# nizepart/Research-and-Development-of-Kubernetes-Operator-for-Machine-Learning-Pipelines

Measured on AMD Instinct MI355X. Metric: served_tokens_per_sec, higher is better.
Workload: dtype bf16

## Files before the change

### research-and-development-of-kubernetes-operator-for-machine-learning-pipelines_amd/ops/csrc/bindings.cpp

```cpp
#include <cstdlib>
#include <string>
#include <torch/library.h>
#include <ATen/ATen.h>
#include <c10/hip/HIPStream.h>
#include <c10/core/DeviceGuard.h>
#include <cmath>

#include "launch.h"
#include "gemm_plan.h"

namespace {

using at::Tensor;

hipStream_t cur_stream() { return c10::hip::getCurrentHIPStream().stream(); }

void check_bf16(const Tensor& t, const char* name) {
  TORCH_CHECK(t.is_cuda(), name, " must be a GPU tensor");
  TORCH_CHECK(t.scalar_type() == at::kBFloat16, name, " must be bf16");
  TORCH_CHECK(t.is_contiguous(), name, " must be contiguous");
}
void check_i32(const Tensor& t, const char* name) {
  TORCH_CHECK(t.is_cuda(), name, " must be a GPU tensor");
  TORCH_CHECK(t.scalar_type() == at::kInt, name, " must be int32");
// ... 281 lines not shown
Tensor vmm_arena(int64_t bytes, int64_t device) {
  void* base = nullptr;
  long reserved = 0;
  std::shared_ptr<void> owner = mlop::vmm_reserve((long)bytes, (int)device, &base, &reserved);
  TORCH_CHECK(owner != nullptr, "hipMemAddressReserve failed");
  const at::Device dev(at::kCUDA, (int)device);
  return at::for_blob(base, {(int64_t)reserved})
      .deleter([owner, base](void*) mutable {
        mlop::vmm_forget(base);
        owner.reset();
      })
      .options(at::TensorOptions().dtype(at::kByte).device(dev))
      .target_device(dev)
      .make_tensor();
}

bool vmm_map_chunks(Tensor flat, int64_t region_stride, int64_t n_regions, int64_t chunk_bytes, int64_t first,
                    int64_t count, bool async) {
  return mlop::vmm_map_chunks(flat.data_ptr(), (long)region_stride, (int)n_regions, (long)chunk_bytes,
                              (long)first, (long)count, async);
}
int64_t vmm_chunks_ready(Tensor flat) { return mlop::vmm_chunks_ready(flat.data_ptr()); }
int64_t vmm_error(Tensor flat) { return mlop::vmm_error(flat.data_ptr()); }

template <int (*F)(int)>
int64_t knob(int64_t set) { return F((int)set); }

void gemm_dense_plan(int64_t variant, int64_t bm, int64_t bn, int64_t splits, int64_t stages) {
  mlop::gemm_dense_plan((int)variant, (int)bm, (int)bn, (int)splits, (int)stages);
}
void gemm_grouped_plan(int64_t bm, int64_t bn, int64_t stages, int64_t splits) {
  mlop::gemm_grouped_plan((int)bm, (int)bn, (int)stages, (int)splits);
}
bool gemm_sk_reserve() { return mlop::gemm_sk_reserve(); }

int64_t gemm_sk_workgroups(int64_t M, int64_t N, int64_t K) {
  return mlop::gemm_sk_workgroups(mlop::gemm_live_env(), (int)M, (int)N, (int)K);
}
int64_t gemm_workspace(int64_t M, int64_t N, int64_t K, int64_t epi) {
  return mlop::gemm_workspace_floats(mlop::gemm_live_env(), (int)M, (int)N, (int)K, epi == 2 ? 0 : (int)epi);
}
bool gemm_rope_supported(int64_t M, int64_t N, int64_t K) {
  return mlop::gemm_rope_supported(mlop::gemm_live_env(), (int)M, (int)N, (int)K);
}
bool w4_chain_ok(int64_t M, int64_t N, int64_t K) { return mlop::w4_chain_ok(mlop::gemm_live_env(), (int)M, (int)N, (int)K); }
bool mid_chain_ok(int64_t M, int64_t N, int64_t K, int64_t epi) {
  return mlop::mid_chain_ok(mlop::gemm_live_env(), (int)M, (int)N, (int)K, (int)epi);
}
bool gemv_chain_supported(int64_t M, int64_t N, int64_t K, int64_t epi) {
  return mlop::decode_chain_takes(mlop::gemm_live_env(), (int)M, (int)N, (int)K, (int)epi);
}
bool chain_ok(int64_t M, int64_t N, int64_t K, int64_t epi) {
  return mlop::chain_ok(mlop::gemm_live_env(), (int)M, (int)N, (int)K, (int)epi);
}
int64_t decode_chain_max_m() { return mlop::decode_chain_max_m(mlop::gemm_live_env()); }

std::vector<int64_t> route_list(const mlop::PlanEnv& env, int64_t M, int64_t N, int64_t K, int64_t op,
                                int64_t n_groups, int64_t rows_per_group) {
  mlop::GemmCall c;
  c.op = (int)op, c.M = (int)M, c.N = (int)N, c.K = (int)K;
  c.n_groups = (int)n_groups, c.rows_per_group = (int)rows_per_group;
  long f[mlop::kRouteFields];
  mlop::gemm_route_fields(mlop::gemm_route(env, c), f);
  return std::vector<int64_t>(f, f + mlop::kRouteFields);
}
std::vector<int64_t> gemm_route(int64_t M, int64_t N, int64_t K, int64_t op, int64_t n_groups, int64_t rows_per_group) {
  return route_list(mlop::gemm_live_env(), M, N, K, op, n_groups, rows_per_group);
}
std::vector<int64_t> gemm_route_env(int64_t M, int64_t N, int64_t K, int64_t op, int64_t cus, bool sk,
                                    int64_t n_groups, int64_t rows_per_group) {
  mlop::PlanEnv env = mlop::gemm_knobs();
  env.cus = (int)cus, env.sk = sk;
  return route_list(env, M, N, K, op, n_groups, rows_per_group);
}
std::vector<int64_t> gemm_tile_configs() {
  std::vector<int64_t> v;
  for (const mlop::TileCfg& t : mlop::kGemmTiles) v.insert(v.end(), {t.BM, t.BN, t.WM, t.WN, t.stages, t.setprio, t.rope});
  return v;
}

void check_a(const Tensor& a) {
  TORCH_CHECK(a.is_cuda() && a.scalar_type() == at::kBFloat16 && a.dim() == 2 && a.stride(1) == 1 &&
                  a.stride(0) % 8 == 0, "a must be bf16 [M, K], 16-B aligned rows");
}

mlop::RopeEpi rope_args(const Tensor& q_out, const Tensor& k_cache, const Tensor& v_cache, const Tensor& a,
                        const Tensor& w, const Tensor& pos, const Tensor& cos_sin, const Tensor& slots) {
  check_a(a);
  check_bf16(w, "w"); check_bf16(q_out, "q_out"); check_bf16(k_cache, "k_cache");
  check_bf16(v_cache, "v_cache"); check_i32(pos, "pos"); check_i32(slots, "slots");
  TORCH_CHECK(cos_sin.is_cuda() && cos_sin.scalar_type() == at::kFloat && cos_sin.is_contiguous(),
              "cos_sin f32");
  const int64_t M = a.size(0), K = a.size(1), N = w.size(0);
  TORCH_CHECK(w.dim() == 2 && w.size(1) == K && K % 64 == 0, "w [N, K], K % 64");
  TORCH_CHECK(q_out.dim() == 3 && k_cache.dim() == 4 && v_cache.dim() == 4, "ranks");
  const int64_t Hq = q_out.size(1), D = q_out.size(2), Hkv = k_cache.size(1), BS = k_cache.size(2);
  TORCH_CHECK(D == 128 && k_cache.size(3) == D && v_cache.sizes() == k_cache.sizes(),
              "head_dim 128; k and v [NB,Hkv,BS,D]");
  TORCH_CHECK(N == (Hq + 2 * Hkv) * D && q_out.size(0) == M, "qkv width / q_out rows");
  TORCH_CHECK(pos.numel() == M && slots.numel() == M, "pos/slots length");
  TORCH_CHECK(cos_sin.dim() == 2 && cos_sin.size(1) == D, "cos_sin [max_pos, D]");
  return mlop::RopeEpi{(uint16_t*)q_out.data_ptr(), (uint16_t*)k_cache.data_ptr(),
                       (uint16_t*)v_cache.data_ptr(), pos.data_ptr<int>(), cos_sin.data_ptr<float>(),
                       slots.data_ptr<int>(), (int)Hq, (int)Hkv, (int)BS};
}

// ... 517 lines not shown

TORCH_LIBRARY(mlop, m) {
  m.def("src_hash() -> str", &src_hash);
  m.def("device_delay(int us) -> ()", &device_delay);
  m.def("car_create(int rank, int world, int max_bytes, int device, bool split=False) -> int", &car_create);
  m.def("car_ipc_handle(int h) -> Tensor", &car_ipc_handle);
  m.def("car_open(int h, Tensor handles) -> ()", &car_open);
  m.def("car_all_reduce(int h, Tensor(a!) out, Tensor inp, bool two_shot=False) -> ()");
  m.def("car_all_reduce_add(int h, Tensor(a!) residual, Tensor inp) -> ()");
  m.def("car_broadcast(int h, Tensor(a!) buf, int root) -> ()");
  m.def("car_all_gather(int h, Tensor(a!) out, Tensor piece) -> ()");
  m.def("car_error(int h) -> int", &car_error);
  m.def("attn_fused_max_pairs(int n) -> int", &attn_fused_max_pairs);
  m.def("car_mem_mode(int h) -> int", &car_mem_mode);
  m.def("car_destroy(int h) -> ()", &car_destroy);
  m.def("chan_create(str name, int slots, int consumers) -> int", &chan_create);
  m.def("chan_open(str name) -> int", &chan_open);
  m.def("chan_send(int h, Tensor vals, int timeout_us) -> bool", &chan_send);
  m.def("chan_recv(int h, int consumer, Tensor(a!) out, int timeout_us) -> bool", &chan_recv);
  m.def("chan_unlink(str name) -> ()", &chan_unlink);
  m.def("chan_close(int h, bool unlink) -> ()", &chan_close);
  m.def("xg_create(str name, int world, int slots, int max_words) -> int", &xg_create);
  m.def("xg_open(str name, int rank) -> int", &xg_open);
  m.def("xg_exchange(int h, Tensor vals, Tensor(a!) out, Tensor(b!) counts, int timeout_us) -> bool", &xg_exchange);
  m.def("xg_close(int h) -> ()", &xg_close);
  m.def("ep_create(int rank, int world, int E, int k, int H, int tcap, int device) -> int", &ep_create);
  m.def("ep_ipc_handle(int h) -> Tensor", &ep_ipc_handle);
  m.def("ep_open(int h, Tensor handles) -> ()", &ep_open);
  m.def("ep_dispatch(int h, Tensor(a!) xp, Tensor(b!) offsets, Tensor x, Tensor topi) -> ()");
  m.def("ep_combine(int h, Tensor(a!) out, Tensor y, Tensor topw, Tensor topi) -> ()");
  m.def("ep_error(int h) -> int", &ep_error);
  m.def("ep_mem_mode(int h) -> int", &ep_mem_mode);
  m.def("ep_destroy(int h) -> ()", &ep_destroy);
  m.def("gemm_workspace(int M, int N, int K, int epi) -> int", &gemm_workspace);
  m.def("gemm_big_variant(int set=-1) -> int", &knob<mlop::gemm_big_variant>);
  m.def("gemm_half_tile(int set=-1) -> int", &knob<mlop::gemm_half_tile>);
  m.def("gemm_small_nt(int set=-1) -> int", &knob<mlop::gemm_small_nt>);
  m.def("attn_kv_nt(int set=-1) -> int", &knob<mlop::attn_kv_nt>);
  m.def("gemm_slab_nt(int set=-1) -> int", &knob<mlop::gemm_slab_nt>);
  m.def("gemm_rope_split(int set=-1) -> int", &knob<mlop::gemm_rope_split>);
  m.def("gemm_split_target(int set=-1) -> int", &knob<mlop::gemm_split_target>);
  m.def("gemm_grouped_narrow(int set=-1) -> int", &knob<mlop::gemm_grouped_narrow>);
  m.def("gemm_ws_max_m(int set=-1) -> int", &knob<mlop::gemm_ws_max_m>);
  m.def("decode_chain_max_m() -> int", &decode_chain_max_m);
  m.def("gemm_ws_plan(int rb, int u, int nt) -> ()", &gemm_ws_plan);
  m.def("gemm_ws_small_m(int set=-1) -> int", &knob<mlop::gemm_ws_small_m>);
  m.def("gemm_ws_rope_m(int set=-1) -> int", &knob<mlop::gemm_ws_rope_m>);
  m.def("flash_persist(int set=-1) -> int", &knob<mlop::flash_persist>);
  m.def("flash_stream(int set=-1) -> int", &knob<mlop::flash_stream>);
  m.def("gemm_grouped_balance(int set=-1) -> int", &knob<mlop::gemm_grouped_balance>);
  m.def("gemm_grouped_order(int set=-1) -> int", &knob<mlop::gemm_grouped_order>);
  m.def("moe_mid_tok(int set=-1) -> int", &knob<mlop::moe_mid_tok>);
  m.def("gemm_mid_chain(int set=-1) -> int", &knob<mlop::gemm_mid_chain>);
  m.def("mid_chain_ok(int M, int N, int K, int epi) -> bool", &mid_chain_ok);
  m.def("moe_mid_max_tokens(int set=-1) -> int", &knob<mlop::moe_mid_max_tokens>);
  m.def("gemm_grouped_plan(int bm, int bn, int stages, int splits) -> ()", &gemm_grouped_plan);
  m.def("gemm_dense_plan(int variant, int bm, int bn, int splits, int stages=0) -> ()", &gemm_dense_plan);
  m.def("gemm_small_stages(int set=-1) -> int", &knob<mlop::gemm_small_stages>);
  m.def("gemm_small_tile(int set=-1) -> int", &knob<mlop::gemm_small_tile>);
  m.def("gemm_sk_mode(int set=-1) -> int", &knob<mlop::gemm_sk_mode>);
  m.def("gemm_sk_reserve() -> bool", &gemm_sk_reserve);
  m.def("gemm_sk_workgroups(int M, int N, int K) -> int", &gemm_sk_workgroups);
  m.def("vmm_supported(int device) -> bool", &vmm_supported);
  m.def("vmm_granularity(int device) -> int", &vmm_granularity);
  m.def("vmm_arena(int bytes, int device) -> Tensor", &vmm_arena);
  m.def("vmm_map_chunks(Tensor flat, int region_stride, int n_regions, int chunk_bytes, int first, "
        "int count, bool async_) -> bool", &vmm_map_chunks);
  m.def("vmm_chunks_ready(Tensor flat) -> int", &vmm_chunks_ready);
  m.def("vmm_error(Tensor flat) -> int", &vmm_error);
  m.def("gemm_rope_supported(int M, int N, int K) -> bool", &gemm_rope_supported);
  m.def("w4_chain_ok(int M, int N, int K) -> bool", &w4_chain_ok);
  m.def("chain_ok(int M, int N, int K, int epi) -> bool", &chain_ok);
  m.def("gemm_route(int M, int N, int K, int op, int n_groups=0, int rows_per_group=0) -> int[]", &gemm_route);
  m.def("gemm_route_env(int M, int N, int K, int op, int cus, bool sk, int n_groups=0, int rows_per_group=0) -> int[]", &gemm_route_env);
  m.def("gemm_tile_configs() -> int[]", &gemm_tile_configs);
  m.def("gemm_res_ss(Tensor(a!) residual, Tensor a, Tensor w, Tensor(b!) ss_out) -> bool");
  m.def("gemm_rs(Tensor(a!) out, Tensor a, Tensor w, Tensor ss_in, float eps, int epi) -> bool");
  m.def("gemm_rs_rope(Tensor(a!) q_out, Tensor(b!) k_cache, Tensor(c!) v_cache, Tensor a, Tensor w, "
        "Tensor pos, Tensor cos_sin, Tensor slots, Tensor ss_in, float eps) -> bool");
  m.def("gemm_rope_cache(Tensor(a!) q_out, Tensor(b!) k_cache, Tensor(c!) v_cache, Tensor a, Tensor w, "
        "Tensor pos, Tensor cos_sin, Tensor slots) -> bool");
  m.def("gemm(Tensor(a!) out, Tensor a, Tensor w, Tensor(b!) ws, int epi) -> ()");
  m.def("grouped_gemm(Tensor(a!) out, Tensor a, Tensor w, Tensor offsets, int max_rows, "
        "int epi, Tensor? a_rows=None) -> ()");
  m.def("gemm_add_rmsnorm(Tensor(a!) out, Tensor(b!) residual, Tensor a, Tensor w, Tensor norm_w, "
        "Tensor(c!) ws, float eps) -> bool");
  m.def("gemv_chain_supported(int M, int N, int K, int epi) -> bool", &gemv_chain_supported);
  m.def("moe_route(Tensor(a!) topw, Tensor(b!) topi, Tensor logits) -> ()");
  m.def("moe_permute(Tensor(a!) xp, Tensor(b!) offsets, Tensor(c!) src, Tensor(d!) inv, Tensor x, "
        "Tensor topi, int e0, int n_local) -> ()");
  m.def("moe_combine(Tensor(a!) out, Tensor y, Tensor inv, Tensor topw) -> ()");
  m.def("moe_dispatch_small(Tensor(a!) topw, Tensor(b!) topi, Tensor(c!) xp, Tensor(d!) offsets, Tensor(e!) src, "
        "Tensor(f!) inv, Tensor(g!) x, Tensor router_w, int e0, int n_local, Tensor? pro_y=None, "
        "Tensor(h!)? pro_res=None, Tensor? pro_w=None, float pro_eps=0.0) -> bool");
  m.def("moe_dispatch_mid(Tensor(a!) topw, Tensor(b!) topi, Tensor(c!) offsets, Tensor(d!) arow, Tensor(e!) inv, "
        "Tensor(f!) x, Tensor router_w, int e0, int n_local, Tensor? pro_y=None, Tensor(g!)? pro_res=None, "
        "Tensor? pro_w=None, float pro_eps=0.0) -> bool");
  m.def("moe_down_combine_add_rmsnorm(Tensor(a!) out, Tensor(b!) residual, Tensor(c!) y, Tensor a, Tensor w2, "
        "Tensor offsets, int max_rows, Tensor inv, Tensor topw, Tensor norm_w, float eps) -> bool");
  m.def("moe_combine_add_rmsnorm(Tensor(a!) out, Tensor(b!) residual, Tensor y, Tensor inv, Tensor topw, "
        "Tensor norm_w, float eps) -> bool");
  m.def("argmax(Tensor(a!) out, Tensor logits) -> ()");
  m.def("sample(Tensor(a!) out, Tensor logits, Tensor temps, Tensor top_ks, Tensor top_ps, "
        "Tensor uniform, bool full) -> ()");
  m.def("penalty_reset(Tensor(a!) table, int slot, int vocab, Tensor prompt_ids, Tensor output_ids) -> ()");
  m.def("penalty_update(Tensor(a!) table, int vocab, Tensor slots, Tensor tokens) -> ()");
// ... 69 lines not shown
```

### research-and-development-of-kubernetes-operator-for-machine-learning-pipelines_amd/ops/csrc/gemm.hip

```cpp
#include "common.h"
#include "launch.h"
#include "gemm_plan.h"
#include "rope_epi.h"

#include <stdexcept>

namespace mlop {

enum { EPI_NONE = 0, EPI_SILU_MUL = 1, EPI_ROPE = 3 };
constexpr int kStages = 3;

__device__ __forceinline__ int swz(int r) { return (r >> 1) & 7; }



template <int AUX>
__device__ __forceinline__ u32x4 ld_b128(__amdgpu_buffer_rsrc_t rs, uint32_t off) {
  return __builtin_bit_cast(u32x4, __builtin_amdgcn_raw_buffer_load_b128(rs, off, 0, AUX));
}
template <int AUX>
__device__ __forceinline__ float ld_f32(__amdgpu_buffer_rsrc_t rs, uint32_t off) {
  return __uint_as_float(__builtin_amdgcn_raw_buffer_load_b32(rs, off, 0, AUX));
}

// ... 957 lines not shown
}

template <int EPI, bool GROUPED>
static void launch_route(const Route& rt, const uint16_t* A, int lda, const uint16_t* B, int ldb, uint16_t* C,
                         int ldc, float* ws, int M, int N, int K, const int* offsets, int n_groups,
                         hipStream_t st, const RopeEpi& re = RopeEpi{}) {
  if (rt.family == FAM_PP) return run_pp<EPI, GROUPED>(rt, A, lda, B, ldb, C, ldc, M, N, K, st, re, offsets, n_groups);
  if ((rt.family == FAM_W4 || rt.family == FAM_W4H) && !GROUPED) {
    if (!run_w4(EPI, A, lda, B, ldb, C, ldc, M, N, K, st, re, rt.BM)) throw std::runtime_error("gemm: four-wave launch refused");
    return;
  }
#define MLOP_GEMM(bm_, bn_, wm_, wn_, st_, prio_, rope_)                                                  \
  if constexpr (EPI != EPI_ROPE || rope_) {                                                               \
    if (rt.family == FAM_TILE && rt.BM == bm_ && rt.BN == bn_ && rt.WM == wm_ && rt.WN == wn_ &&          \
        rt.stages == st_ && rt.setprio == (int)prio_)                                                     \
      return run_cfg<bm_, bn_, wm_, wn_, EPI, GROUPED, st_, prio_>(A, lda, B, ldb, C, ldc, ws, M, N, K,   \
                                                                   rt.splits, rt.k_chunk, offsets,        \
                                                                   n_groups, rt.m_tiles, st, re);         \
  }
  MLOP_GEMM_TILES(MLOP_GEMM)
#undef MLOP_GEMM
  throw std::runtime_error("gemm: the route names no kernel built for this epilogue");
}

static GemmCall gemm_call(int op, int M, int N, int K, int lda, int ldb, int ldc) {
  GemmCall c;
  c.op = op, c.M = M, c.N = N, c.K = K, c.lda = lda, c.ldb = ldb, c.ldc = ldc;
  return c;
}

static void launch_splitk_reduce(int epi, uint16_t* C, int ldc, const float* ws, int M, int N, int splits,
                                 hipStream_t st, const int* m_valid = nullptr) {
  const int outw = epi == EPI_NONE ? N : N / 2;
  const long total = (long)M * (outw / 8);
  const int g = (int)std::min<long>((total + 255) / 256, 4096);
  if (epi == EPI_NONE) splitk_reduce_kernel<EPI_NONE><<<g, 256, 0, st>>>(C, ldc, ws, M, N, splits, m_valid);
  else splitk_reduce_kernel<EPI_SILU_MUL><<<g, 256, 0, st>>>(C, ldc, ws, M, N, splits, m_valid);
}

static void run_rope_route(const Route& rt, const void* A, int lda, const void* B, int M, int N, int K,
                           const RopeEpi& re, hipStream_t st) {
  if (rt.family == FAM_GEMV) return launch_gemv_rope(A, lda, B, M, N, K, re, st);
  if (rt.family == FAM_WS) return launch_ws(A, lda, B, K, nullptr, 0, M, N, K, EPI_ROPE, false, re, 0.f, st);
  if (rt.finish == FIN_ROPE_SLABS) {
    float* ws = sk_buf()->ws;
    launch_route<EPI_NONE, false>(rt, (const uint16_t*)A, lda, (const uint16_t*)B, K, nullptr, N, ws, M, N, K,
                                  nullptr, 0, st);
    return launch_rope_cache_slabs(re, ws, rt.splits, M, N, st);
  }
  launch_route<EPI_ROPE, false>(rt, (const uint16_t*)A, lda, (const uint16_t*)B, K, nullptr, 0, nullptr, M, N, K,
                                nullptr, 0, st, re);
}

bool launch_gemm_rope(const void* A, int lda, const void* B, int M, int N, int K, const RopeEpi& re,
                      hipStream_t st) {
  if (M == 0) return true;
  const Route rt = gemm_route(gemm_live_env(), gemm_call(OP_ROPE, M, N, K, lda, K, 0));
  if (!rt.ok()) return false;
  run_rope_route(rt, A, lda, B, M, N, K, re, st);
  return true;
}

bool launch_gemm_chain(int op, const void* A, int lda, const void* B, void* C, int ldc, int M, int N, int K,
                       const RopeEpi& rope, float* ss, float eps, hipStream_t st) {
  const PlanEnv env = gemm_live_env();
  const Route rt = gemm_route(env, gemm_call(op, M, N, K, lda, K, ldc));
  if (!rt.ok()) return false;
  const bool res = op == OP_CHAIN_RES_SS;
  const int epi = res ? EPI_NONE : op & 3;
  RopeEpi re = epi == EPI_ROPE ? rope : RopeEpi{};
  if (M <= decode_chain_max_m(env)) {
    if (rt.family == FAM_GEMV && res) launch_gemv_res(A, lda, B, C, M, N, K, st);
    else if (rt.family == FAM_GEMV) launch_gemv_rs(A, lda, B, C, ldc, M, N, K, epi, re, eps, st);
    else if (res) launch_ws(A, lda, B, K, C, N, M, N, K, 5, false, re, 0.f, st);
    else launch_ws(A, lda, B, K, C, ldc, M, N, K, epi, true, re, eps, st);
    return true;
  }
  if (res) {
    re.ss_out = ss;
    re.ss_tot = ss + (size_t)M * (N / 128);
  } else {
    re.ss_in = ss + (size_t)M * (K / 128);
    re.ss_inv_k = 1.f / (float)K;
    re.ss_eps = eps;
  }
  if (rt.family == FAM_W4 || rt.family == FAM_W4H)
    return run_w4(res ? 4 : epi | 8, (const uint16_t*)A, lda, (const uint16_t*)B, K, (uint16_t*)C, ldc, M, N, K, st, re, rt.BM);
  if (epi == EPI_ROPE) {
    if (rt.family == FAM_WS) launch_ws(A, lda, B, K, nullptr, 0, M, N, K, 3, true, re, eps, st);
    else run_rope_route(rt, A, lda, B, M, N, K, re, st);
    return true;
  }
  if (res) {
    float* ws = nullptr;
    int cus = 0;
    RopeEpi fin{};
    if (!gemm_sk_scratch(&ws, &fin.ss_cnt, &cus)) return false;
    fin.ss_tot = re.ss_tot;
    fin.mid_acq = env.mid_chain == 2;
    launch_route<EPI_NONE, false>(rt, (const uint16_t*)A, lda, (const uint16_t*)B, K, (uint16_t*)C, ldc, ws, M, N, K,
                                  nullptr, 0, st, fin);
    return true;
  }
  RopeEpi rs{};
  rs.ss_in = re.ss_in;
  rs.ss_inv_k = re.ss_inv_k;
  rs.ss_eps = eps;
  launch_route<EPI_SILU_MUL, false>(rt, (const uint16_t*)A, lda, (const uint16_t*)B, K, (uint16_t*)C, ldc, nullptr, M,
                                    N, K, nullptr, 0, st, rs);
  return true;
}

void launch_gemm(const void* A, int lda, const void* B, int ldb, void* C, int ldc, float* ws,
                 long ws_floats, int M, int N, int K, int epi, hipStream_t st) {
  if (M == 0) return;
  GemmCall c = gemm_call(epi, M, N, K, lda, ldb, ldc);
  c.ws_avail = ws_floats;
  const Route rt = gemm_route(gemm_live_env(), c);
// ... 72 lines not shown
```

### research-and-development-of-kubernetes-operator-for-machine-learning-pipelines_amd/ops/csrc/gemm_plan.cc

```cpp
#include "gemm_plan.h"

#include <algorithm>
#include <stddef.h>
#include <stdexcept>

namespace mlop {

namespace {
enum { EPI_NONE = 0, EPI_SILU_MUL = 1, EPI_ROPE = 3 };
enum { WS_NONE = 0, WS_SILU_MUL = 1, WS_ROPE = 3, WS_RES = 5 };
constexpr int kHeadD = 128;
constexpr int kGroupedSmallStages = 3;
}

static PlanEnv g_knobs;
PlanEnv& gemm_knobs() { return g_knobs; }

int gemm_split_target(int set) {
  if (set >= 1) g_knobs.split_target = set;
  return g_knobs.split_target;
}

int gemm_small_stages(int set) {
  if (set >= 0) g_knobs.small_stages = set;
// ... 406 lines not shown
    if (env.sk_on() && s > 1 && (size_t)s * M * N * 4 <= (size_t)kSkScratchFloats * 4) {
      p.splits = s;
      p.k_chunk = K / s;
    }
  }
  const Route r = resolve(env, p, M, N, K, true, false, false);
  return r.family == FAM_TILE && r.splits > 1 ? with_slabs(r, FIN_REDUCE, WS_SRC_SCRATCH, M, N) : r;
}

Route route_chain(const PlanEnv& env, const GemmCall& c, int lda, int ldc) {
  const int M = c.M, N = c.N, K = c.K;
  const int epi = c.op == OP_CHAIN_RES_SS ? EPI_NONE : c.op & 3;
  if (M <= decode_chain_max_m(env)) {
    if ((c.op == OP_CHAIN_RES_SS && ldc != N) || !decode_chain_takes(env, M, N, K, epi)) return refused();
    return simple(M <= env.gemv_chain_max_m ? FAM_GEMV : FAM_WS);
  }
  const Plan base = plan(env, M, N, K, false, 0, 0);
  const Plan p = epi == EPI_ROPE ? rope_split(env, base, K) : base;
  if (mid_chain_plan_ok(env, p, M, N, K, epi)) {
    if (epi == EPI_ROPE) {
      return ws_prefer(env, M, N, K, EPI_ROPE) ? simple(FAM_WS) : route_rope(env, c, lda);
    }
    if (c.op == OP_CHAIN_RS) return refused();
    Route r = resolve(env, p, M, N, K, false, false, false);
    if (epi == EPI_NONE) { r.ws_src = WS_SRC_SCRATCH; r.ws_floats = (long)r.splits * M * N; }
    return r;
  }
  if (!w4_chain_plan_ok(env, base, M, N, K) || !gemm_w4_ok(M, N, K, lda, K, ldc)) return refused();
  return w4_route(base.BM);
}

}

Route gemm_route(const PlanEnv& env, const GemmCall& c) {
  if (c.M <= 0) return refused();
  const bool silu = c.op == OP_SILU_MUL || c.op == OP_GROUPED_SILU || c.op == OP_CHAIN_RS_SILU;
  const int lda = c.lda ? c.lda : c.K, ldb = c.ldb ? c.ldb : c.K;
  const int ldc = c.ldc ? c.ldc : c.op == OP_ROPE || c.op == OP_CHAIN_RS_ROPE ? 0 : silu ? c.N / 2 : c.N;
  switch (c.op) {
    case OP_PLAIN:
    case OP_SILU_MUL: return route_plain(env, c, lda, ldb, ldc);
    case OP_ADD_RMSNORM: return route_add_rmsnorm(env, c, lda);
    case OP_ROPE: return route_rope(env, c, lda);
    case OP_CHAIN_RES_SS:
    case OP_CHAIN_RS:
    case OP_CHAIN_RS_SILU:
    case OP_CHAIN_RS_ROPE: return route_chain(env, c, lda, ldc);
    case OP_GROUPED:
    case OP_GROUPED_SILU: return route_grouped(env, c);
    default: throw std::runtime_error("gemm_route: unknown op");
  }
}

void gemm_route_fields(const Route& r, long out[kRouteFields]) {
  const long f[kRouteFields] = {r.family, r.tile,   r.BM,      r.BN,    r.WM,   r.WN,     r.stages, r.setprio,
                                r.splits, r.k_chunk, r.m_tiles, r.sk_d, r.sk_wgs, r.finish, r.ws_src, r.ws_floats};
  std::copy(f, f + kRouteFields, out);
}


static GemmCall call(int op, int M, int N, int K) {
  GemmCall c;
  c.op = op, c.M = M, c.N = N, c.K = K;
  return c;
}

bool gemm_rope_supported(const PlanEnv& e, int M, int N, int K) { return gemm_route(e, call(OP_ROPE, M, N, K)).ok(); }

bool w4_chain_ok(const PlanEnv& e, int M, int N, int K) {
  return M > 0 && w4_chain_plan_ok(e, plan(e, M, N, K, false, 0, 0), M, N, K);
}

bool mid_chain_ok(const PlanEnv& e, int M, int N, int K, int epi) {
  if (!mid_chain_rows(e, M, N, K)) return false;
  return mid_chain_plan_ok(e, epi == EPI_ROPE ? rope_plan(e, M, N, K) : plan(e, M, N, K, false, 0, 0), M, N, K, epi);
}

bool chain_ok(const PlanEnv& e, int M, int N, int K, int epi) {
  if (M <= decode_chain_max_m(e)) return decode_chain_takes(e, M, N, K, epi < 0 ? EPI_NONE : epi);
  if (M <= 64 && epi >= 0) return mid_chain_ok(e, M, N, K, epi);
  return w4_chain_ok(e, M, N, K);
}

long gemm_workspace_floats(const PlanEnv& e, int M, int N, int K, int epi) {
  const Route r = gemm_route(e, call(epi == EPI_SILU_MUL ? OP_SILU_MUL : OP_PLAIN, M, N, K));
  return r.ws_src == WS_SRC_CALLER ? r.ws_floats : 0;
}

int gemm_sk_workgroups(const PlanEnv& e, int M, int N, int K) {
  const Route r = gemm_route(e, call(OP_PLAIN, M, N, K));
  return r.family == FAM_PP ? r.sk_wgs : 0;
}

}
```

### research-and-development-of-kubernetes-operator-for-machine-learning-pipelines_amd/ops/csrc/gemm_plan.h

```cpp
#pragma once

#if defined(__HIP__) || defined(__HIPCC__)
#define MLOP_HD __host__ __device__
#else
#define MLOP_HD
#endif

namespace mlop {

constexpr int kBK = 64;
constexpr int kMaxSplits = 8;
constexpr int kSkMaxWg = 256;
constexpr long kSkScratchFloats = 2l * kSkMaxWg * 256 * 256;
constexpr int kSkMinIters = 16;
constexpr int sk_min_half() { return kSkMinIters / 2 > 1 ? kSkMinIters / 2 : 1; }

MLOP_HD inline int sk_choose_d(int T, int nk, int cus, int min_half) {
  const int r = T % cus;
  if (r == 0) return 0;
  float best = 0.9f * nk;
  int best_d = 0;
  const int dmax = cus / r < 32 ? cus / r : 32;
  for (int d = 2; d <= dmax; ++d) {
    if (nk % d || nk / d < min_half) continue;
    const float w = 0.04f * r * d;
    const float cost = nk / d + (w > 2.f ? w : 2.f) + 2.f * (d >= 3 ? d : d - 1) + 1.f;
    if (cost < best) {
      best = cost;
      best_d = d;
    }
  }
  return best_d;
}

struct PlanEnv {
  int cus = 0;
  bool sk = false;
  int small_tile = 1;
  int small_stages = 3;
  int big_variant = 5;
  int half_tile = 1;
  int grouped_narrow = 1;
  int split_target = 512;
  int rope_split_k = 2;
  int sk_mode = 1;
  int mid_chain = 0;
  int gp[4] = {-1, -1, -1, -1};
  int dp[5] = {-1, -1, -1, -1, 0};
  int ws_small_m = 8, ws_rope_m = 8, ws_max_m = 0;
  int gemv_max_m = 4, gemv_chain_max_m = 4;
  bool sk_on() const { return sk_mode && sk && cus > 0; }
};
PlanEnv& gemm_knobs();
PlanEnv gemm_live_env();
int gemm_small_tile(int set);
int gemm_small_stages(int set);
int gemm_big_variant(int set);
int gemm_half_tile(int set);
int gemm_grouped_narrow(int set);
int gemm_split_target(int set);
int gemm_rope_split(int set);
int gemm_sk_mode(int set);
int gemm_mid_chain(int set);
int gemm_ws_small_m(int set);
int gemm_ws_rope_m(int set);
int gemm_ws_max_m(int set);

enum GemmOp {
  OP_PLAIN = 0,
  OP_SILU_MUL = 1,
  OP_ADD_RMSNORM = 2,
  OP_ROPE = 3,
  OP_CHAIN_RES_SS = 4,
  OP_CHAIN_RS = 8,
  OP_CHAIN_RS_SILU = 9,
  OP_CHAIN_RS_ROPE = 11,
  OP_GROUPED = 16,
  OP_GROUPED_SILU = 17,
};

struct GemmCall {
  int op = OP_PLAIN;
  int M = 0, N = 0, K = 0;
  int lda = 0, ldb = 0, ldc = 0;
  int n_groups = 0, rows_per_group = 0;
  long ws_avail = -1;
  bool indirect = false;
};

enum GemmFamily { FAM_REFUSED = 0, FAM_GEMV, FAM_WS, FAM_TILE, FAM_PP, FAM_W4, FAM_W4H };
enum GemmFinish { FIN_NONE = 0, FIN_REDUCE, FIN_ADD_RMSNORM, FIN_ROPE_SLABS, FIN_RMSNORM };
enum GemmWsSrc { WS_SRC_NONE = 0, WS_SRC_CALLER, WS_SRC_SCRATCH };

#define MLOP_GEMM_TILES(X)       \
  X(16, 32, 1, 2, 8, false, 0)   \
  X(16, 32, 1, 2, 6, false, 0)   \
  X(16, 32, 1, 2, 4, false, 0)   \
  X(16, 64, 1, 2, 8, false, 0)   \
  X(16, 64, 1, 2, 6, false, 0)   \
  X(16, 64, 1, 2, 4, false, 0)   \
  X(32, 32, 1, 2, 8, false, 0)   \
  X(32, 32, 1, 2, 4, false, 0)   \
  X(32, 64, 1, 4, 6, false, 0)   \
  X(32, 64, 1, 4, 4, false, 0)   \
  X(64, 32, 1, 2, 4, false, 0)   \
  X(64, 64, 1, 4, 6, false, 0)   \
  X(64, 64, 1, 4, 4, false, 0)   \
  X(64, 64, 1, 4, 3, false, 0)   \
  X(128, 64, 2, 2, 5, false, 0)  \
  X(128, 64, 2, 2, 3, false, 0)  \
  X(256, 64, 4, 2, 3, false, 0)  \
  X(256, 128, 4, 2, 3, false, 1) \
  X(256, 256, 2, 4, 2, true, 1)  \
  X(256, 256, 2, 4, 2, false, 1)

struct TileCfg {
  int BM, BN, WM, WN, stages;
  bool setprio, rope;
};
#define MLOP_TILE_ENTRY(bm, bn, wm, wn, st, prio, rope) {bm, bn, wm, wn, st, prio, rope != 0},
constexpr TileCfg kGemmTiles[] = {MLOP_GEMM_TILES(MLOP_TILE_ENTRY)};
#undef MLOP_TILE_ENTRY
constexpr int kNumGemmTiles = sizeof(kGemmTiles) / sizeof(kGemmTiles[0]);

struct Route {
  int family = FAM_REFUSED;
  int tile = -1;
  int BM = 0, BN = 0, WM = 0, WN = 0, stages = 0, setprio = 0;
  int splits = 1, k_chunk = 0;
  int m_tiles = 0;
  int sk_d = 0, sk_wgs = 0;
  int finish = FIN_NONE;
  int ws_src = WS_SRC_NONE;
  long ws_floats = 0;
  bool ok() const { return family != FAM_REFUSED; }
};
constexpr int kRouteFields = 16;
void gemm_route_fields(const Route& r, long out[kRouteFields]);

Route gemm_route(const PlanEnv& env, const GemmCall& c);

void gemm_grouped_plan(int bm, int bn, int stages, int splits);
void gemm_dense_plan(int variant, int bm, int bn, int splits, int stages);

bool gemv_takes(const PlanEnv& e, int M, int N, int K, int epi);
bool gemv_chain_takes(const PlanEnv& e, int M, int N, int K, int epi);
bool gemv_grouped_takes(int M, int N, int K, int epi);
bool ws_takes(const PlanEnv& e, int M, int N, int K, int epi);
bool ws_prefer(const PlanEnv& e, int M, int N, int K, int epi);
int decode_chain_max_m(const PlanEnv& e);
bool decode_chain_takes(const PlanEnv& e, int M, int N, int K, int epi);
bool gemm_w4_ok(int M, int N, int K, int lda, int ldb, int ldc);
bool gemm_w4_split_ok(const PlanEnv& e, int T, int nk);
bool sk_halves_ok(const PlanEnv& e, long T, int nk);
bool gemm_rope_supported(const PlanEnv& e, int M, int N, int K);
bool w4_chain_ok(const PlanEnv& e, int M, int N, int K);
bool mid_chain_ok(const PlanEnv& e, int M, int N, int K, int epi);
bool chain_ok(const PlanEnv& e, int M, int N, int K, int epi);
long gemm_workspace_floats(const PlanEnv& e, int M, int N, int K, int epi);
int gemm_sk_workgroups(const PlanEnv& e, int M, int N, int K);

}
```

### research-and-development-of-kubernetes-operator-for-machine-learning-pipelines_amd/ops/csrc/gemm_w4.hip

```cpp
#include "common.h"
#include "launch.h"
#include "gemm_plan.h"
#include "gemm_w4_asm.h"

#include <type_traits>
#include <utility>

namespace mlop {

namespace {
enum { W4_NONE = 0, W4_SILU_MUL = 1, W4_ROPE = 3, W4_ADD_SS = 4, W4_RS = 8 };
using i32x4 = __attribute__((ext_vector_type(4))) int;
typedef __attribute__((address_space(3))) uint16_t lds_u16;

__device__ __forceinline__ i32x4 make_srd(const void* p) {
  const uint64_t a = (uint64_t)p;
  i32x4 r;
  r.x = __builtin_amdgcn_readfirstlane((int)(uint32_t)a);
  r.y = __builtin_amdgcn_readfirstlane((int)(uint32_t)(a >> 32));
  r.z = 0x7fffffff;
  r.w = 0x00020000;
  return r;
}

// ... 199 lines not shown
        const int tk = __hip_atomic_fetch_add(cnt + tt, 1, __ATOMIC_RELAXED, __HIP_MEMORY_SCOPE_AGENT);
        if (tk == 1) __hip_atomic_store(cnt + tt, 0, __ATOMIC_RELAXED, __HIP_MEMORY_SCOPE_AGENT);
        flag[0] = tk == 1;
      }
      __syncthreads();
      const int last = flag[0];
      __syncthreads();
      if (!last) break;
    }
    auto fetch = [&](auto I_, float (&v)[32]) {
      constexpr int I = decltype(I_)::value;
      read_block<I>(v);
      if (part) {
#pragma unroll
        for (int b4 = 0; b4 < 8; b4 += 4) {
          u32x4 o[4];
#pragma unroll
          for (int q4 = 0; q4 < 4; ++q4)
            o[q4] = __builtin_bit_cast(u32x4, __builtin_amdgcn_raw_buffer_load_b128(
                                                  rs_other, (uint32_t)(((I * 8 + b4 + q4) * 256 + tid) * 16), 0, 16 ));
#pragma unroll
          for (int q4 = 0; q4 < 4; ++q4)
#pragma unroll
            for (int e = 0; e < 4; ++e) v[4 * (b4 + q4) + e] += __uint_as_float(o[q4][e]);
        }
      }
      if constexpr (RS) {
        const float f = rsqrtf(rinv_lds[wid * 128 + 16 * I + (lane & 15)] * re.ss_inv_k + re.ss_eps);
#pragma unroll
        for (int e = 0; e < 32; ++e) v[e] *= f;
      }
    };
    const int odd = qd & 1, half = qd >> 1;
    auto swap_f = [&](const float* x, const float* y, float (&lo)[4], float (&hi)[4]) {
#pragma unroll
      for (int r = 0; r < 4; ++r) {
        const auto sw2 = __builtin_amdgcn_permlane16_swap(__float_as_uint(x[r]), __float_as_uint(y[r]), false, false);
        lo[r] = __uint_as_float(sw2[0]);
        hi[r] = __uint_as_float(sw2[1]);
      }
    };
    auto swap_pair = [&](const float* x, const float* y, u32x4& out) {
      float lo[4], hi[4];
      swap_f(x, y, lo, hi);
      out = u32x4{pack2(lo[0], lo[1]), pack2(lo[2], lo[3]), pack2(hi[0], hi[1]), pack2(hi[2], hi[3])};
    };
    if constexpr (BASE == W4_ROPE) {
      constexpr int D = 128, HALF = 64;
      const bool r_nt = (re.ws_nt & 8) != 0;
      auto put16 = [&](uint16_t* p, const u32x4& v) {
        if (r_nt) __builtin_nontemporal_store(v, reinterpret_cast<u32x4*>(p));
        else *reinterpret_cast<u32x4*>(p) = v;
      };
      const int head = (n0 + wn * 128) / D;
      const int n_rope = re.Hq + re.Hkv, n_all = re.Hq + 2 * re.Hkv;
      if (head >= n_all) {
      } else if (head >= n_rope) {
        const int kh = head - n_rope;
        int sl[NI];
#pragma unroll
        for (int I = 0; I < NI; ++I) {
          const int m = m0 + lr + I * 16;
          sl[I] = m < M ? re.slots[m] : -1;
        }
        auto vstore = [&](auto I_) {
          constexpr int I = decltype(I_)::value;
          float v[32];
          fetch(I_, v);
          u32x4 d[4];
#pragma unroll
          for (int pr = 0; pr < 4; ++pr) swap_pair(v + 8 * pr, v + 8 * pr + 4, d[pr]);
          const int slot = sl[I];
          if (slot < 0) return;
          uint16_t* dst = re.v_cache + (((size_t)(slot / re.BS) * re.Hkv + kh) * re.BS + slot % re.BS) * D;
#pragma unroll
          for (int pr = 0; pr < 4; ++pr)
            put16(dst + (2 * pr + odd) * 16 + 8 * half, d[pr]);
        };
        unroll<NI>(vstore);
      } else {
        const bool is_k = head >= re.Hq;
        int pp[NI], sl[NI];
#pragma unroll
        for (int I = 0; I < NI; ++I) {
          const int m = m0 + lr + I * 16;
          const bool ok = m < M;
          pp[I] = ok ? re.pos[m] : 0;
          sl[I] = ok && is_k ? re.slots[m] : -1;
        }
        const int c0 = 4 * qd;
        auto load_cs = [&](int I, float4 (&cs)[8]) {
          const float4* cr = reinterpret_cast<const float4*>(re.cos_sin + (size_t)pp[I] * D);
#pragma unroll
          for (int j = 0; j < 4; ++j) {
            cs[j] = cr[(j * 16 + c0) / 4];
            cs[4 + j] = cr[(HALF + j * 16 + c0) / 4];
          }
        };
        auto rstore = [&](auto I_, const float4 (&cs)[8], float4 (&nxt)[8]) {
          constexpr int I = decltype(I_)::value;
          if constexpr (I < NI - 1) load_cs(I + 1, nxt);
          float v[32];
          fetch(I_, v);
          float xo[4][4], yo[4][4];
#pragma unroll
          for (int j = 0; j < 4; ++j) {
            const float cv[4] = {cs[j].x, cs[j].y, cs[j].z, cs[j].w};
// ... 225 lines not shown
```

### research-and-development-of-kubernetes-operator-for-machine-learning-pipelines_amd/ops/csrc/launch.h

```cpp
#pragma once

#include <string>
#include <hip/hip_runtime.h>
#include <stdint.h>
#include <algorithm>
#include <memory>

namespace mlop {

void launch_rmsnorm(void* out, const void* x, const void* w, float eps, int M, int H,
                    hipStream_t st);
void launch_add_rmsnorm(void* out, void* residual, const void* x, const void* w, float eps, int M,
                        int H, hipStream_t st);
void launch_rope_cache(void* q_out, void* k_cache, void* v_cache, const void* qkv, const int* pos,
                       const float* cos_sin, const int* slots, int T, int Hq, int Hkv, int D,
                       int qkv_stride, int BS, hipStream_t st);
void launch_silu_mul(void* out, const void* x, int M, int I, int interleaved, hipStream_t st);
void launch_device_delay(long long ticks, hipStream_t st);
void launch_lora_shrink(const void* x, int ldx, const void* A, float* tmp, const int* tok_slot,
                        const int* slot_rank, int T, int K, int GR, int R, int S, hipStream_t st);
void launch_lora_expand_add(void* y, int ldy, const float* tmp, const void* B, const uint8_t* tile_group,
                            const int* tok_slot, const int* slot_rank, int T, int N, int GR, int R, int S,
                            hipStream_t st);
void launch_embedding(void* out, const void* table, const long* ids, int T, int H, long vocab_start,
                      long vocab_end, hipStream_t st);
void launch_paged_attention(void* out, float* part_o, float* part_ml, const void* q,
                            const void* kc, const void* vc, const int* bt, int bt_stride,
                            const int* tile_seq, const int* tile_q0, const int* q_start,
                            const int* q_len, const int* ctx_len, int num_tiles, int Hq, int Hkv,
                            float scale_log2, int part_tokens, int nparts, int num_blocks,
                            int* sem, int window, hipStream_t st);
void launch_rope_cache_fp8(void* q_out, void* k_cache, void* v_cache, void* k_scale, void* v_scale,
                           const void* qkv, const int* pos, const float* cos_sin, const int* slots, int T,
                           int Hq, int Hkv, int qkv_stride, int BS, hipStream_t st);
void launch_paged_attention_fp8(void* out, float* part_o, float* part_ml, const void* q, const void* kc,
                                const void* vc, const void* ks, const void* vs, const int* bt,
                                int bt_stride, const int* tile_seq, const int* tile_q0, const int* q_start,
                                const int* q_len, const int* ctx_len, int num_tiles, int Hq, int Hkv,
                                float scale_log2, int part_tokens, int nparts, int num_blocks, int* sem,
                                hipStream_t st);
int flash_persist(int set);
int flash_stream(int set);
int gemm_grouped_balance(int set);
int gemm_grouped_order(int set);
int moe_mid_tok(int set);
void launch_flash_prefill(void* out, const void* q, const void* kc, const void* vc, const int* bt,
                          int bt_stride, const int* ptile_seq, const int* ptile_q0,
                          const int* q_start, const int* q_len, const int* ctx_len, int num_ptiles,
                          int Hq, int Hkv, float scale_log2, int num_blocks, int window, hipStream_t st);
struct RopeEpi {
  uint16_t* q_out;
  uint16_t* k_cache;
  uint16_t* v_cache;
  const int* pos;
  const float* cos_sin;
  const int* slots;
  int Hq, Hkv, BS;
  const float* ss_in = nullptr;
  float* ss_out = nullptr;
  float* ss_tot = nullptr;
  int* ss_cnt = nullptr;
  float ss_inv_k = 0.f, ss_eps = 0.f;
  const int* a_rows = nullptr;
  int b_nt = 0;
  int ws_nt = 0;
  int mid_acq = 0;
};
void launch_rope_cache_slabs(const RopeEpi& re, const float* ws, int splits, int T, int N, hipStream_t st);
bool gemm_sk_scratch(float** ws, int** cnt, int* cus);
bool gemm_sk_available(int* cus);
bool run_w4(int epi, const uint16_t* A, int lda, const uint16_t* B, int ldb, uint16_t* C, int ldc, int M, int N,
            int K, hipStream_t st, const RopeEpi& re, int bm = 256);
bool launch_gemm_chain(int op, const void* A, int lda, const void* B, void* C, int ldc, int M, int N, int K,
                       const RopeEpi& rope, float* ss, float eps, hipStream_t st);
int gemm_small_nt(int set);
int attn_kv_nt(int set);
int gemm_slab_nt(int set);
bool gemm_sk_reserve();
void launch_gemv(const void* A, int lda, const void* B, int ldb, void* C, int ldc, int M, int N, int K,
                 int epi, hipStream_t st);
void launch_gemv_rope(const void* A, int lda, const void* B, int M, int N, int K, const RopeEpi& re,
                      hipStream_t st);
struct NormPro {
  float eps = 0.f;
};
void gemm_ws_plan(int rb, int u, int nt);
void launch_ws(const void* A, int lda, const void* B, int ldb, void* C, int ldc, int M, int N, int K, int epi,
               bool rs, const RopeEpi& re, float eps, hipStream_t st);
void launch_gemv_rs(const void* A, int lda, const void* B, void* C, int ldc, int M, int N, int K, int epi,
                    const RopeEpi& re, float eps, hipStream_t st);
void launch_gemv_res(const void* A, int lda, const void* B, void* residual, int M, int N, int K, hipStream_t st);
void launch_gemv_grouped(const void* A, const void* B, void* C, const int* offsets, int n_groups, int M, int N,
                         int K, int epi, hipStream_t st);
bool launch_gemm_rope(const void* A, int lda, const void* B, int M, int N, int K, const RopeEpi& re,
                      hipStream_t st);
void launch_gemm(const void* A, int lda, const void* B, int ldb, void* C, int ldc, float* ws,
                 long ws_floats, int M, int N, int K, int epi, hipStream_t st);
bool launch_gemm_add_rmsnorm(const void* A, int lda, const void* B, void* out, void* residual,
                             const void* w, float eps, float* ws, long ws_floats, int M, int N,
                             int K, hipStream_t st);
void launch_grouped_gemm(const void* A, const void* B, void* C, const int* offsets, int n_groups,
                         int M, int N, int K, int max_rows, int epi, hipStream_t st, const int* a_rows = nullptr,
                         float** defer_ws = nullptr, int* defer_splits = nullptr);
bool launch_moe_down_combine_add_rmsnorm(void* out, void* residual, void* y, const void* a, const void* w2,
                                         const int* offsets, int n_groups, int R, int H, int I, int max_rows,
                                         const int* inv, const float* topw, const void* norm_w, float eps, int T,
                                         int k, hipStream_t st);
bool moe_dispatch_mid_takes(int T, int E, int k, int H);
int moe_mid_max_tokens(int set);
void launch_moe_dispatch_mid(float* topw, int* topi, int* offsets, int* arow, int* inv, const void* x, const void* wr,
// ... 83 lines not shown
```

Before: 38390.

## Split fused QKV rope GEMM into separate Q and KV four-wave launches

When the whole QKV projection's tile count does not divide evenly across CUs, the QKV+rope GEMM is split column-wise into a Q part and a KV part, each launched as its own four-wave kernel with its own BM. A head0 offset is added to the rope epilogue so the KV launch writes to the right heads. The goal is to cut wave-quantization tail loss on prefill-sized QKV GEMMs. The trade-off is an extra kernel launch and possibly lower A-tile reuse. The split is gated by a heuristic and is on by default.

```diff
diff --git a/research-and-development-of-kubernetes-operator-for-machine-learning-pipelines_amd/ops/csrc/bindings.cpp b/research-and-development-of-kubernetes-operator-for-machine-learning-pipelines_amd/ops/csrc/bindings.cpp
--- a/research-and-development-of-kubernetes-operator-for-machine-learning-pipelines_amd/ops/csrc/bindings.cpp
+++ b/research-and-development-of-kubernetes-operator-for-machine-learning-pipelines_amd/ops/csrc/bindings.cpp
@@ -357,6 +357,9 @@
 }
 bool chain_ok(int64_t M, int64_t N, int64_t K, int64_t epi) {
   return mlop::chain_ok(mlop::gemm_live_env(), (int)M, (int)N, (int)K, (int)epi);
+}
+int64_t qkv_col_split(int64_t M, int64_t N, int64_t K, int64_t q_cols, int64_t op) {
+  return mlop::qkv_col_split(mlop::gemm_live_env(), (int)M, (int)N, (int)K, (int)q_cols, (int)op);
 }
 int64_t decode_chain_max_m() { return mlop::decode_chain_max_m(mlop::gemm_live_env()); }
 
@@ -980,6 +983,8 @@
   m.def("gemm_grouped_order(int set=-1) -> int", &knob<mlop::gemm_grouped_order>);
   m.def("moe_mid_tok(int set=-1) -> int", &knob<mlop::moe_mid_tok>);
   m.def("gemm_mid_chain(int set=-1) -> int", &knob<mlop::gemm_mid_chain>);
+  m.def("gemm_qkv_split(int set=-1) -> int", &knob<mlop::gemm_qkv_split>);
+  m.def("qkv_col_split(int M, int N, int K, int q_cols, int op=3) -> int", &qkv_col_split);
   m.def("mid_chain_ok(int M, int N, int K, int epi) -> bool", &mid_chain_ok);
   m.def("moe_mid_max_tokens(int set=-1) -> int", &knob<mlop::moe_mid_max_tokens>);
   m.def("gemm_grouped_plan(int bm, int bn, int stages, int splits) -> ()", &gemm_grouped_plan);
diff --git a/research-and-development-of-kubernetes-operator-for-machine-learning-pipelines_amd/ops/csrc/gemm.hip b/research-and-development-of-kubernetes-operator-for-machine-learning-pipelines_amd/ops/csrc/gemm.hip
--- a/research-and-development-of-kubernetes-operator-for-machine-learning-pipelines_amd/ops/csrc/gemm.hip
+++ b/research-and-development-of-kubernetes-operator-for-machine-learning-pipelines_amd/ops/csrc/gemm.hip
@@ -1033,10 +1033,27 @@
                                 nullptr, 0, st, re);
 }
 
+static bool run_w4_qkv_split(const PlanEnv& env, int op, int epi, const void* A, int lda, const void* B, int M, int N,
+                             int K, const RopeEpi& re, hipStream_t st) {
+  int bm_q = 0, bm_kv = 0;
+  const int q_cols = qkv_col_split(env, M, N, K, re.Hq * 128, op, lda, &bm_q, &bm_kv);
+  if (q_cols <= 0) return false;
+  RopeEpi kv = re;
+  kv.head0 = re.Hq;
+  const uint16_t* a = (const uint16_t*)A;
+  const uint16_t* b = (const uint16_t*)B;
+  if (!run_w4(epi, a, lda, b + (size_t)q_cols * K, K, nullptr, 0, M, N - q_cols, K, st, kv, bm_kv) ||
+      !run_w4(epi, a, lda, b, K, nullptr, 0, M, q_cols, K, st, re, bm_q))
+    throw std::runtime_error("gemm: four-wave launch refused");
+  return true;
+}
+
 bool launch_gemm_rope(const void* A, int lda, const void* B, int M, int N, int K, const RopeEpi& re,
                       hipStream_t st) {
   if (M == 0) return true;
-  const Route rt = gemm_route(gemm_live_env(), gemm_call(OP_ROPE, M, N, K, lda, K, 0));
+  const PlanEnv env = gemm_live_env();
+  if (run_w4_qkv_split(env, OP_ROPE, EPI_ROPE, A, lda, B, M, N, K, re, st)) return true;
+  const Route rt = gemm_route(env, gemm_call(OP_ROPE, M, N, K, lda, K, 0));
   if (!rt.ok()) return false;
   run_rope_route(rt, A, lda, B, M, N, K, re, st);
   return true;
@@ -1045,6 +1062,13 @@
 bool launch_gemm_chain(int op, const void* A, int lda, const void* B, void* C, int ldc, int M, int N, int K,
                        const RopeEpi& rope, float* ss, float eps, hipStream_t st) {
   const PlanEnv env = gemm_live_env();
+  if (op == OP_CHAIN_RS_ROPE && M > 0) {
+    RopeEpi rs = rope;
+    rs.ss_in = ss + (size_t)M * (K / 128);
+    rs.ss_inv_k = 1.f / (float)K;
+    rs.ss_eps = eps;
+    if (run_w4_qkv_split(env, op, EPI_ROPE | 8, A, lda, B, M, N, K, rs, st)) return true;
+  }
   const Route rt = gemm_route(env, gemm_call(op, M, N, K, lda, K, ldc));
   if (!rt.ok()) return false;
   const bool res = op == OP_CHAIN_RES_SS;
diff --git a/research-and-development-of-kubernetes-operator-for-machine-learning-pipelines_amd/ops/csrc/gemm_plan.cc b/research-and-development-of-kubernetes-operator-for-machine-learning-pipelines_amd/ops/csrc/gemm_plan.cc
--- a/research-and-development-of-kubernetes-operator-for-machine-learning-pipelines_amd/ops/csrc/gemm_plan.cc
+++ b/research-and-development-of-kubernetes-operator-for-machine-learning-pipelines_amd/ops/csrc/gemm_plan.cc
@@ -482,6 +482,47 @@
   }
 }
 
+int gemm_qkv_split(int set) {
+  if (set >= 0) g_knobs.qkv_split = set > 2 ? 2 : set;
+  return g_knobs.qkv_split;
+}
+
+int qkv_col_split(const PlanEnv& env, int M, int N, int K, int q_cols, int op, int lda, int* bm_q, int* bm_kv) {
+  if (!env.qkv_split || (op != OP_ROPE && op != OP_CHAIN_RS_ROPE)) return 0;
+  if (M <= 0 || q_cols <= 0 || q_cols >= N || q_cols % 256 || K % kBK) return 0;
+  const int ld = lda ? lda : K, n_kv = N - q_cols;
+  GemmCall c;
+  c.op = op, c.M = M, c.K = K, c.lda = ld;
+  const bool rule = env.qkv_split == 1;
+  if (rule) {
+    if (env.cus <= 0) return 0;
+    const int T = ((M + 255) / 256) * ((N + 255) / 256);
+    if (T % env.cus == 0 || !gemm_w4_split_ok(env, T, K / kBK)) return 0;
+    c.N = N;
+    const Route whole = gemm_route(env, c);
+    if (whole.family != FAM_W4 || whole.BM != 256) return 0;
+  }
+  c.N = q_cols;
+  const Route rq = gemm_route(env, c);
+  c.N = n_kv;
+  const Route rkv = gemm_route(env, c);
+  const bool q_w4 = rq.family == FAM_W4 || rq.family == FAM_W4H, kv_w4 = rkv.family == FAM_W4 || rkv.family == FAM_W4H;
+  const int hq = q_w4 ? rq.BM : 256, hkv = kv_w4 ? rkv.BM : 128;
+  if (!rule) {
+    if (M <= 64) return 0;
+    if (!gemm_w4_ok(M, q_cols, K, ld, K, 0) || !gemm_w4_ok(M, n_kv, K, ld, K, 0)) return 0;
+  } else {
+    const int t_q = ((M + 255) / 256) * (q_cols / 256);
+    if (rq.family != FAM_W4 || t_q % env.cus) return 0;
+    if (!kv_w4) return 0;
+    const long t_kv = (long)((M + hkv - 1) / hkv) * (n_kv / 256), rounds = (t_kv + env.cus - 1) / env.cus;
+    if (8 * t_kv < 7 * rounds * env.cus) return 0;
+  }
+  if (bm_q) *bm_q = hq;
+  if (bm_kv) *bm_kv = hkv;
+  return q_cols;
+}
+
 void gemm_route_fields(const Route& r, long out[kRouteFields]) {
   const long f[kRouteFields] = {r.family, r.tile,   r.BM,      r.BN,    r.WM,   r.WN,     r.stages, r.setprio,
                                 r.splits, r.k_chunk, r.m_tiles, r.sk_d, r.sk_wgs, r.finish, r.ws_src, r.ws_floats};
diff --git a/research-and-development-of-kubernetes-operator-for-machine-learning-pipelines_amd/ops/csrc/gemm_plan.h b/research-and-development-of-kubernetes-operator-for-machine-learning-pipelines_amd/ops/csrc/gemm_plan.h
--- a/research-and-development-of-kubernetes-operator-for-machine-learning-pipelines_amd/ops/csrc/gemm_plan.h
+++ b/research-and-development-of-kubernetes-operator-for-machine-learning-pipelines_amd/ops/csrc/gemm_plan.h
@@ -45,6 +45,7 @@
   int rope_split_k = 2;
   int sk_mode = 1;
   int mid_chain = 0;
+  int qkv_split = 1;
   int gp[4] = {-1, -1, -1, -1};
   int dp[5] = {-1, -1, -1, -1, 0};
   int ws_small_m = 8, ws_rope_m = 8, ws_max_m = 0;
@@ -62,6 +63,7 @@
 int gemm_rope_split(int set);
 int gemm_sk_mode(int set);
 int gemm_mid_chain(int set);
+int gemm_qkv_split(int set);
 int gemm_ws_small_m(int set);
 int gemm_ws_rope_m(int set);
 int gemm_ws_max_m(int set);
@@ -140,6 +142,9 @@
 
 Route gemm_route(const PlanEnv& env, const GemmCall& c);
 
+int qkv_col_split(const PlanEnv& env, int M, int N, int K, int q_cols, int op = OP_ROPE, int lda = 0,
+                  int* bm_q = nullptr, int* bm_kv = nullptr);
+
 void gemm_grouped_plan(int bm, int bn, int stages, int splits);
 void gemm_dense_plan(int variant, int bm, int bn, int splits, int stages);
 
diff --git a/research-and-development-of-kubernetes-operator-for-machine-learning-pipelines_amd/ops/csrc/gemm_w4.hip b/research-and-development-of-kubernetes-operator-for-machine-learning-pipelines_amd/ops/csrc/gemm_w4.hip
--- a/research-and-development-of-kubernetes-operator-for-machine-learning-pipelines_amd/ops/csrc/gemm_w4.hip
+++ b/research-and-development-of-kubernetes-operator-for-machine-learning-pipelines_amd/ops/csrc/gemm_w4.hip
@@ -275,7 +275,7 @@
         if (r_nt) __builtin_nontemporal_store(v, reinterpret_cast<u32x4*>(p));
         else *reinterpret_cast<u32x4*>(p) = v;
       };
-      const int head = (n0 + wn * 128) / D;
+      const int head = re.head0 + (n0 + wn * 128) / D;
       const int n_rope = re.Hq + re.Hkv, n_all = re.Hq + 2 * re.Hkv;
       if (head >= n_all) {
       } else if (head >= n_rope) {
diff --git a/research-and-development-of-kubernetes-operator-for-machine-learning-pipelines_amd/ops/csrc/launch.h b/research-and-development-of-kubernetes-operator-for-machine-learning-pipelines_amd/ops/csrc/launch.h
--- a/research-and-development-of-kubernetes-operator-for-machine-learning-pipelines_amd/ops/csrc/launch.h
+++ b/research-and-development-of-kubernetes-operator-for-machine-learning-pipelines_amd/ops/csrc/launch.h
@@ -56,6 +56,7 @@
   const float* cos_sin;
   const int* slots;
   int Hq, Hkv, BS;
+  int head0 = 0;
   const float* ss_in = nullptr;
   float* ss_out = nullptr;
   float* ss_tot = nullptr;
```

Result: no change. 38380 (-0.0%).
